# EllarBooher/Syzygy

Hardware: AMD Instinct MI355X
Metric: Mpixels/s deferred-lit+atmosphere (higher is better)
Workload: dtype f32

## Files before the change

syzygy_amd/csrc/kernels_composite.hip:

```cpp

#include "szg_device.hpp"
#include "szg_launch.hpp"

namespace szg
{
namespace
{
template <typename T> SZG_DEV T* row_ptr(const szg_image& im, unsigned y)
{
    return reinterpret_cast<T*>(static_cast<unsigned char*>(im.data) + (size_t)y * im.pitch_bytes);
}

struct SkyLut
{
    const float4* texels;
    int width, height;
    bool finite;
};

SZG_DEV V3 sampleMapDirection(const SkyLut& S, const Atm& a, V3 position, V3 direction)
{
    float const PI = 3.141592653589793f;
    V3 const normalized = normalize(direction);
    float const sinHorizonZenith = a.planetRadius / length(position);
    float const horizonZenith = PI - szg_asinf(sinHorizonZenith);
    float const cosViewZenith = normalized.y;
    float const cosHorizonZenith = -safeSqrt(1.0f - sinHorizonZenith * sinHorizonZenith);
    float const viewZenith = szg_acosf(normalized.y);
    float v;
    if (cosViewZenith > cosHorizonZenith)
    {
        float const angleFraction = viewZenith / horizonZenith;
        v = (1.0f - sqrtf(1.0f - angleFraction)) * 0.5f;
    }
    else
    {
        float const angleFraction = (viewZenith - horizonZenith) / (PI - horizonZenith);
        v = sqrtf(angleFraction) * 0.5f + 0.5f;
    }
    V2 const projectedLight = normalize(V2{-a.incidentDirectionSun.x, -a.incidentDirectionSun.z});
    V2 const projectedView = normalize(V2{direction.x, direction.z});
    float const u = clampf(dot(projectedLight, projectedView), -1.0f, 1.0f) * 0.5f + 0.5f;
    return bilinear_rgb(S.texels, S.width, S.height, (float)S.width, (float)S.height, u, v);
}

SZG_DEV V3 sampleSunDisk(const TLut& L, const Atm& a, V3 position, V3 direction)
{
    V3 const directionToSun = -a.incidentDirectionSun;
    float const cosDirectionSun = dot(direction, directionToSun) / (length(direction) * length(directionToSun));
    float const sinSunRadius = a.sunAngularRadius;
    float const sinDirectionSun = safeSqrt(1.0f - cosDirectionSun * cosDirectionSun);
    if (cosDirectionSun < 0.0f)
    {
        return splat(0.0f);
    }
    V3 const transmittanceToSun = sampleT_Ray(L, a, position, direction);
    return transmittanceToSun * (1.0f - smoothstep(0.2f * sinSunRadius, sinSunRadius, sinDirectionSun));
}

SZG_DEV bool raycastGround(const Atm& a, V3 origin, V3 direction, float& distance)
{
    float t0 = 0.0f, t1 = 0.0f;
    bool const hit = raySphere(origin, direction, a.planetRadius, t0, t1) && t0 > 0.0f;
    distance = t0;
    return hit;
}

SZG_DEV V3 groundSurfaceTerm(const TLut& L, const Atm& a, V3 origin, V3 direction, float distanceToGround)
{
    float const PI = 3.141592653589793f;
    V3 const surfacePosition = origin + distanceToGround * direction;
    V3 const surfaceNormal = normalize(surfacePosition);
    V3 const lightDirection = -a.incidentDirectionSun;
    V3 const viewDirection = -direction;
    V3 const h = normalize(lightDirection + viewDirection);
    float const specularPower = 160.0f;
    float const microfacet = szg_powf(clampf(dot(h, surfaceNormal), 0.0f, 1.0f), specularPower);
    float const normalization = (specularPower + 2.0f) / 8.0f;
    V3 const specular = splat(normalization * microfacet);
    V3 const diffuse = splat(0.4f) / PI;
    V3 const fresnel =
        splat(0.04f) + (splat(1.0f) - splat(0.04f)) * szg_powf(1.0f - clampf(dot(h, lightDirection), 0.0f, 1.0f), 5.0f);
    V3 const albedo = mix(diffuse, specular, fresnel);
    V3 const transmittanceToSun = sampleT_Ray(L, a, surfacePosition, lightDirection);
    V3 const surfaceLuminance = (transmittanceToSun * albedo) * clampf(dot(surfaceNormal, lightDirection), 0.0f, 1.0f);
    V3 const transmittanceToSurface = sampleT_Segment(L, a, origin, surfacePosition);
    return surfaceLuminance * transmittanceToSurface;
}
}

#ifdef SZG_TAIL_DIAG
__device__ unsigned long long* g_tailStamps = nullptr;
extern "C" int szg_debug_tail_buffer(void* d_buffer)
{
    return (int)hipMemcpyToSymbol(HIP_SYMBOL(g_tailStamps), &d_buffer, sizeof d_buffer);
}
struct TailStamp
{
    unsigned long long start;
    unsigned slot;
    SZG_DEV TailStamp(unsigned slot_) : start(wall_clock64()), slot(slot_) {}
// ... 71 lines not shown
    }
    unsigned const gy = global_row(rm, y);

    Atm const a = load_atm(*prep);
#ifdef SZG_EXP_LDS_TLUT
    TLut L = make_tlut(tlut, tW, tH, *prep);
    L.ldsRows = tW == 512 ? (const __attribute__((address_space(3))) float*)s_tlutRows : nullptr;
#else
    TLut const L = make_tlut(tlut, tW, tH, *prep);
#endif
    SkyLut const S{slut, sW, sH, reinterpret_cast<const unsigned*>(slut + (size_t)sW * (size_t)sH)[0] == 0u};
    const szg_camera_packed* cam = cameras + cameraIndex;

    float const sceneDepth = row_ptr<const float>(depth, y)[x];

    V3 position = mk3(cam->position[0], cam->position[1], cam->position[2]) / 1000000.0f;
    position.y *= -1.0f;
    position.y += a.planetRadius;

    float const clipx = ((float)x / (float)drawW - 0.5f) * 2.0f;
    float const clipy = ((float)gy / (float)drawH - 0.5f) * 2.0f;
    M4 const inverseProjection = load_m4(cam->inverseProjection);
    M4 const rotation = load_m4(cam->rotation);
    V4 const dvs = mul(inverseProjection, clipx, clipy, 1.0f, 1.0f);
    V4 const rot = mul(rotation, dvs.x, dvs.y, dvs.z, dvs.w);
    V3 direction = normalize(mk3(rot.x, rot.y, rot.z));
    direction.y *= -1.0f;

    bool isSky = (sceneDepth == 0.0f);
    Material m;
    if (!isSky)
    {
        V4 const diffuse = unpack_half4(row_ptr<const uint2>(g.diffuse, y)[x]);
        V4 const specular = unpack_half4(row_ptr<const uint2>(g.specular, y)[x]);
        V4 const normal = unpack_half4(row_ptr<const uint2>(g.normal, y)[x]);
        V4 const orm = unpack_half4(row_ptr<const uint2>(g.orm, y)[x]);
        float4 const p4 = row_ptr<const float4>(g.position, y)[x];
        m = convertPBR(V4{p4.x, p4.y, p4.z, p4.w}, normal, diffuse, specular, orm);
        isSky = m.position.y > 0.0f;
    }

    V3 surfaceLuminance = splat(0.0f);
    V3 base = splat(0.0f);
    V3 coef = splat(0.0f);
    V3 env2 = splat(0.0f);
    bool hasReflection = false;
    bool march0 = false, march1 = false;
    V3 o0 = position, d0 = direction, o1 = position, d1 = direction;
    float l0 = 0.0f, l1 = 0.0f;

    if (isSky)
    {
        float dtg;
        if (raycastGround(a, position, direction, dtg))
        {
            base = groundSurfaceTerm(L, a, position, direction, dtg);
            march0 = true;
            l0 = dtg;
        }
        else
        {
            base = sampleMapDirection(S, a, position, direction) + sampleSunDisk(L, a, position, direction) * 1.0f;
        }
    }
    else
    {
        uint2 const prior = row_ptr<const uint2>(color, y)[x];
        surfaceLuminance = mk3((float)(prior.x & 0xFFFFu) / 65535.0f, (float)(prior.x >> 16) / 65535.0f,
                               (float)(prior.y & 0xFFFFu) / 65535.0f);

        float shadowFactor = 1.0f;
        if (sunSlot.map != nullptr)
        {
            M4 sm;
#pragma unroll
            for (int k = 0; k < 16; k++)
            {
                sm.m[k] = prep->sunShadow[k];
            }
            V4 c = mul(sm, m.position.x, m.position.y, m.position.z, 1.0f);
            float const w = c.w;
            V3 const coord = mk3(c.x / w, c.y / w, c.z / w);
            V4 const pn = mul(sm, m.normal.x, m.normal.y, m.normal.z, 0.0f);
            float const fdx = sqrtf(1.0f - clampf(pn.x * pn.x, 0.0f, 1.0f));
            float const fdy = sqrtf(1.0f - clampf(pn.y * pn.y, 0.0f, 1.0f));
            shadowFactor = sampleShadowMap(sunSlot.map, sunSlot.width, sunSlot.height, sunSlot.pitchFloats, coord, fdx, fdy);
        }

        m.normal.y *= -1.0f;
        m.position.y *= -1.0f;
        m.position = m.position / 1000000.0f;
        m.position.y += a.planetRadius;

        V3 const surfacePosition = m.position;
        V3 const toSurface = surfacePosition - position;
        bool const samplesLean = waveAll(a.lean && leanRadius2(a, dot(position, position)) && leanRadius2(a, dot(surfacePosition, surfacePosition)) &&
                                         leanLength2(dot(toSurface, toSurface)) &&
                                         leanLength2(dot(a.incidentDirectionSun, a.incidentDirectionSun)));
        V3 const transmittanceToSurface = samplesLean ? sampleT_Segment<true>(L, a, position, surfacePosition)
                                                      : sampleT_Segment<false>(L, a, position, surfacePosition);
        V3 const minusSun = -a.incidentDirectionSun, minusDirection = -direction;
        float const direction2 = dot(minusDirection, minusDirection);
        bool const vectorsLean = samplesLean && waveAll(leanLength2(direction2));
        V3 const lightDirection = vectorsLean ? minusSun * divN0(1.0f, sqrtP(dot(minusSun, minusSun))) : normalize(minusSun);
        V3 const viewDirection = vectorsLean ? minusDirection * divN0(1.0f, sqrtP(direction2)) : normalize(minusDirection);
        float pt0 = 0.0f, pt1 = 0.0f;
        bool const shadowedByPlanet = raySphere(surfacePosition, lightDirection, a.planetRadius, pt0, pt1) && pt0 > 0.0f;
        V3 const halfSum = lightDirection + viewDirection;
        bool const brdfLean = vectorsLean && waveAll(inRange(dot(halfSum, halfSum), 0x1p-40f, 8.0f));
        V3 const brdf = brdfLean ? brdfMix<true>(m, lightDirection, viewDirection) : brdfMix<false>(m, lightDirection, viewDirection);
        V3 const transmittanceToSun = samplesLean ? sampleT_Ray<true>(L, a, surfacePosition, lightDirection)
                                                  : sampleT_Ray<false>(L, a, surfacePosition, lightDirection);
        float const fractionOfSunVisible = vectorsLean ? divN0(a.planetRadius, sqrtP(dot(m.position, m.position)))
                                                       : a.planetRadius / length(m.position);
        float const scalar = (shadowFactor * fractionOfSunVisible) * (shadowedByPlanet ? 0.0f : 1.0f);
        base = ((((scalar * transmittanceToSun) * transmittanceToSurface) * m.occlusion) * brdf) *
               clampf(dot(m.normal, lightDirection), 0.0f, 1.0f);
        l0 = vectorsLean ? sqrtP(dot(toSurface, toSurface)) : length(surfacePosition - position);
        if (FAST)
        {
            base = base + sampleAerial(aerial, (float)x / (float)drawW, (float)gy / (float)drawH, l0);
        }
        else
        {
            march0 = true;
        }

        float const cameraR2 = dot(position, position), surfaceR2 = dot(surfacePosition, surfacePosition);
        float const nBig = 0x1p60f;
        bool const normalFinite = fabsf(m.normal.x) <= nBig && fabsf(m.normal.y) <= nBig && fabsf(m.normal.z) <= nBig;
        float const cameraSinHorizon = vectorsLean ? divN0(a.planetRadius, sqrtP(cameraR2)) : a.planetRadius / length(position);
        bool const aboveGround = cameraSinHorizon <= 1.0f && fractionOfSunVisible <= 1.0f;
        bool const environmentFinite = a.extModerate && a.sunSane && L.moderate && S.finite && normalFinite && aboveGround &&
                                       inRange(cameraR2, a.extFloor2, a.extCeil2) && inRange(surfaceR2, a.extFloor2, a.extCeil2);
        if (m.metallic != 0.0f || !environmentFinite)
        {
            hasReflection = true;
            V3 const negDir = -direction;
            V3 const parallel = dot(m.normal, negDir) * m.normal;
            V3 const reflectionDirection = 2.0f * parallel - negDir;
            coef = (transmittanceToSurface * m.metallic) * computeFresnel(m, negDir, reflectionDirection);
            float dtg2;
            if (raycastGround(a, m.position, reflectionDirection, dtg2))
            {
                env2 = groundSurfaceTerm(L, a, m.position, reflectionDirection, dtg2);
                march1 = true;
                o1 = m.position;
                d1 = reflectionDirection;
                l1 = dtg2;
            }
            else
            {
                env2 = sampleMapDirection(S, a, m.position, reflectionDirection) +
                       sampleSunDisk(L, a, m.position, reflectionDirection) * shadowFactor;
            }
        }
// ... 51 lines not shown
    hasReflection = (flags & 4u) != 0u;
    V3 const ap0 = march0 ? mk3(s_result[0][0][tid], s_result[0][1][tid], s_result[0][2][tid]) : splat(0.0f);
    V3 const ap1 = march1 ? mk3(s_result[1][0][tid], s_result[1][1][tid], s_result[1][2][tid]) : splat(0.0f);
    base = mk3(s_park[0][tid], s_park[1][tid], s_park[2][tid]);
    coef = mk3(s_park[3][tid], s_park[4][tid], s_park[5][tid]);
    env2 = mk3(s_park[6][tid], s_park[7][tid], s_park[8][tid]);
    surfaceLuminance = mk3(s_park[9][tid], s_park[10][tid], s_park[11][tid]);
    V3 transfer = march0 ? (base + ap0) : base;
    if (hasReflection)
    {
        V3 const e2 = march1 ? (env2 + ap1) : env2;
        transfer = transfer + coef * e2;
    }
    V3 const luminance = transfer * mk3(prep->a.sunIntensitySpectrum.x, prep->a.sunIntensitySpectrum.y, prep->a.sunIntensitySpectrum.z);
    V3 const pre = luminance * 10.0f + surfaceLuminance;
    V3 const out = mk3(szg_powf(pre.x, 1.2f), szg_powf(pre.y, 1.2f), szg_powf(pre.z, 1.2f));
    row_ptr<uint2>(color, y)[x] = pack_unorm16x4(out.x, out.y, out.z, 1.0f);
    if (debug.data != nullptr)
    {
        row_ptr<float4>(debug, y)[x] = make_float4(out.x, out.y, out.z, 1.0f);
    }
}

hipError_t launch_composite(hipStream_t s, const szg_scene_texture& scene, unsigned drawW, unsigned drawH, TileArgs tile,
                            const szg_gbuffer& g, ShadowSlot sunSlot, const szg_atmosphere_packed* d_atm, unsigned atmIndex, const szg_camera_packed* d_cam,
                            unsigned camIndex, const szg_directional_light_packed* d_dir, unsigned sunIndex, const float* tlut,
                            unsigned tW, unsigned tH, const float* slut, unsigned sW, unsigned sH, AerialLut aerial, const void* d_prep)
{
    unsigned const rows = tile.nranks <= 1u ? drawH : tile.local_rows;
    if (rows == 0u || drawW == 0u)
    {
// ... 23 lines not shown
```

syzygy_amd/csrc/kernels_deferred.hip:

```cpp

#include "szg_device.hpp"
#include "szg_launch.hpp"

namespace szg
{
namespace
{
SZG_DEV void pixel_of_thread(unsigned& x, unsigned& y)
{
    unsigned const tid = threadIdx.x;
    unsigned const wave = tid >> 6, lane = tid & 63u;
    x = blockIdx.x * 32u + wave * 8u + (lane & 7u);
    y = blockIdx.y * 8u + (lane >> 3);
}
SZG_DEV void pixel_of_thread_bottom_up(unsigned& x, unsigned& y)
{
    unsigned const tid = threadIdx.x;
    unsigned const wave = tid >> 6, lane = tid & 63u;
    x = blockIdx.x * 32u + wave * 8u + (lane & 7u);
    y = (gridDim.y - 1u - blockIdx.y) * 8u + (lane >> 3);
}

template <typename T> SZG_DEV T* row_ptr(const szg_image& im, unsigned y)
{
// ... 454 lines not shown
#endif
    unsigned x, y;
    pixel_of_thread_bottom_up(x, y);
    if (x >= drawW || y >= localRows)
    {
        return;
    }
    V4 const diffuse = unpack_half4(row_ptr<const uint2>(g.diffuse, y)[x]);
    V3 sum = splat(0.0f);
    if (!(diffuse.w < 1.0f))
    {
        V4 const specular = unpack_half4(row_ptr<const uint2>(g.specular, y)[x]);
        V4 const normal = unpack_half4(row_ptr<const uint2>(g.normal, y)[x]);
        V4 const orm = unpack_half4(row_ptr<const uint2>(g.orm, y)[x]);
        float4 const p4 = row_ptr<const float4>(g.position, y)[x];
        Material const m = convertPBR(V4{p4.x, p4.y, p4.z, p4.w}, normal, diffuse, specular, orm);
        const szg_camera_packed* cam = cameras + cameraIndex;
        V3 const viewDirection = normalizeL(mk3(cam->position[0], cam->position[1], cam->position[2]) - m.position);

        float const hi = 0x1p30f;
        bool const positionModerate = fabsf(m.position.x) <= hi && fabsf(m.position.y) <= hi && fabsf(m.position.z) <= hi;
        float const big = 0x1p120f;
        bool const pixelFinite = positionModerate && fabsf(viewDirection.x) <= 2.0f && fabsf(viewDirection.y) <= 2.0f &&
                                 fabsf(viewDirection.z) <= 2.0f && fabsf(m.normal.x) <= big && fabsf(m.normal.y) <= big &&
                                 fabsf(m.normal.z) <= big && fabsf(m.diffuse.x) <= big && fabsf(m.diffuse.y) <= big &&
                                 fabsf(m.diffuse.z) <= big && fabsf(m.reflectance.x) <= big && fabsf(m.reflectance.y) <= big &&
                                 fabsf(m.reflectance.z) <= big && fabsf(m.occlusion) <= big && fabsf(m.normalization) <= big &&
                                 fabsf(m.specularPower) <= big;
        bool const pixelModerate = pixelFinite && fabsf(m.diffuse.x) <= 0x1p16f && fabsf(m.diffuse.y) <= 0x1p16f &&
                                   fabsf(m.diffuse.z) <= 0x1p16f && fabsf(m.reflectance.x) <= 4.0f && fabsf(m.reflectance.y) <= 4.0f &&
                                   fabsf(m.reflectance.z) <= 4.0f && fabsf(m.occlusion) <= 0x1p16f && fabsf(m.normalization) <= 0x1p8f &&
                                   fabsf(m.normal.x) <= 0x1p16f && fabsf(m.normal.y) <= 0x1p16f && fabsf(m.normal.z) <= 0x1p16f;
        bool const waveFinite = waveAll(pixelFinite);
// ... 329 lines not shown
```

syzygy_amd/csrc/kernels_lut.hip:

```cpp

#include "szg_device.hpp"
#include "szg_launch.hpp"

namespace szg
{
template <int CTRL> SZG_DEV float dpp(float v)
{
    return __builtin_bit_cast(float, __builtin_amdgcn_update_dpp(0, __builtin_bit_cast(int, v), CTRL, 0xF, 0xF, false));
}

constexpr int T_LANES = 8;
constexpr int T_STEPS = 500;

template <bool LEAN> SZG_DEV V3 transmittanceProduct(const Atm& a, V3 origin, V3 direction, float distance, float ndt, int sub)
{
    V3 T = splat(1.0f);
    float const rcp500 = rcpN(500.0f);
#pragma unroll 1
    for (int k = 0; k < (T_STEPS + T_LANES - 1) / T_LANES; k++)
    {
        int const i = k * T_LANES + sub;
        float const t = divRX<LEAN>(distance * ((float)i + 0.5f), 500.0f, rcp500);
        V3 const position = origin + t * direction;
        float const altitude = sqrtPX<LEAN>(dotT(position, position)) - a.planetRadius;
// ... 149 lines not shown
        return;
    }
    unsigned const tid = threadIdx.x;
    unsigned const wave = tid >> 6, lane = tid & 63u;
    int const x = (int)(blockIdx.x * 32u + wave * 8u + (lane & 7u));
    int const y = rowBegin + (int)(blockIdx.y * 8u + (lane >> 3));
    if (x >= W || y >= rowEnd)
    {
        return;
    }
    Atm const a = load_atm(*prep);
    TLut const L = make_tlut(tlut, tW, tH, *prep);
    const szg_camera_packed* cam = cameras + cameraIndex;
    float const PI = 3.141592653589793f;

    float const u = ((float)x + 0.5f) / (float)W;
    float const v = ((float)y + 0.5f) / (float)H;

    V3 origin = mk3(cam->position[0], cam->position[1], cam->position[2]) / 1000000.0f;
    origin.y *= -1.0f;
    origin.y += a.planetRadius;

    float const radius = length(origin);
    float const sinHorizonZenith = a.planetRadius / radius;
    float const horizonZenith = PI - szg_asinf(sinHorizonZenith);
    float const cosineViewLightProjected = (u - 0.5f) * 2.0f;
    V2 const lightDirectionProjected = normalize(V2{-a.incidentDirectionSun.x, -a.incidentDirectionSun.z});
    float azimuthSun = szg_asinf(lightDirectionProjected.x);
    if (lightDirectionProjected.y < 0.0f)
    {
        azimuthSun = PI - azimuthSun;
    }
    float const azimuth = szg_acosf(clampf(cosineViewLightProjected, -1.0f, 1.0f)) + azimuthSun;
    float viewZenith;
    float const unnormalized_v = 2.0f * v - 1.0f;
    if (v < 0.5f)
    {
        float const angleFraction = 1.0f - unnormalized_v * unnormalized_v;
        viewZenith = angleFraction * horizonZenith;
    }
    else
    {
        float const angleFraction = unnormalized_v * unnormalized_v;
        viewZenith = (PI - horizonZenith) * angleFraction + horizonZenith;
    }
    float const elevation = -(viewZenith - PI / 2.0f);

    float const ce = szg_cosf(elevation);
    V3 const direction = normalize(mk3(szg_sinf(azimuth) * ce, szg_sinf(elevation), szg_cosf(azimuth) * ce));

    float const distance = raycastAtmosphere(a, origin, direction);
    V3 const luminance = scatteringIntegral(L, a, origin, direction, distance);
    lut[y * W + x] = make_float4(luminance.x, luminance.y, luminance.z, 1.0f);
    if (!slutTexelFinite(luminance.x, luminance.y, luminance.z))
    {
        atomicOr(reinterpret_cast<unsigned*>(lut + (size_t)W * (size_t)H), 1u);
    }
}

__global__ __launch_bounds__(256) void k_slut_check(float4* __restrict__ lut, unsigned n)
{
    unsigned const id = blockIdx.x * 256u + threadIdx.x;
    bool ok = true;
    if (id < n)
    {
        float4 const t = lut[id];
// ... 309 lines not shown
```

syzygy_amd/csrc/szg_device.hpp:

```cpp
#pragma once

#include <hip/hip_fp16.h>
#include <hip/hip_runtime.h>

#include "szg/abi.h"
#include "szg/fpmath.h"

#define SZG_DEV __device__ __forceinline__

namespace szg
{
struct V2
{
    float x, y;
};
struct V3
{
    float x, y, z;
};
struct V4
{
    float x, y, z, w;
};

// ... 116 lines not shown
    u = __builtin_fmaf(u, s, 0.166666671633720397949219f);
    u = __builtin_fmaf(u, s, 0.5f);
    u = __builtin_fmaf(s * s, u, s) + 1.0f;
    return __builtin_ldexpf(u, (int)q);
}
template <bool LEAN> SZG_DEV float divX(float a, float b) { return LEAN ? divR0(a, b, rcpN(b)) : a / b; }
template <bool LEAN> SZG_DEV float divRX(float a, float b, float y) { return LEAN ? divR0(a, b, y) : a / b; }
SZG_DEV float xorSign(float x, unsigned signMask)
{
    return __builtin_bit_cast(float, __builtin_bit_cast(unsigned, x) ^ signMask);
}
SZG_DEV bool slutTexelFinite(float r, float g, float b) { return fabsf(r) <= 0x1p100f && fabsf(g) <= 0x1p100f && fabsf(b) <= 0x1p100f; }
SZG_DEV bool inRange(float x, float lo, float hi) { return x >= lo && x <= hi; }
SZG_DEV float divN0(float a, float b) { return divR0(a, b, rcpN(b)); }
SZG_DEV bool waveAll(bool c) { return __builtin_amdgcn_ballot_w64(!c) == 0ull; }

SZG_DEV float powLean(float x, float y)
{
    int const bits = szg_float_to_bits(x * 1.3333333333333333333333333333333333333f);
    int const e = ((bits >> 23) & 0xFF) - 127;
    float const m = szg_bits_to_float(szg_float_to_bits(x) - (e << 23));
    float const t = szg_div_moderate(m - 1.0f, m + 1.0f);
    float const t2 = t * t;
    float p = 0.2392828464508056640625f;
    p = __builtin_fmaf(p, t2, 0.28518211841583251953125f);
    p = __builtin_fmaf(p, t2, 0.400005877017974853515625f);
    p = __builtin_fmaf(p, t2, 0.666666686534881591796875f);
    p = __builtin_fmaf(p, t2, 2.0f);
    float const fe = (float)e;
    float const lg = __builtin_fmaf(t, p, 0.693147180559945286226764f * fe);
// ... 298 lines not shown
    if (LEAN && a.zeroAbsorptionRayleigh && a.zeroScatteringOzone)
    {
        e.extinction = (scatteringRayleigh + scatteringMie) + absorptionOzone;
    }
    else if (LEAN && a.zeroAbsorptionRayleigh)
    {
        e.extinction = ((scatteringRayleigh + scatteringMie) + scatteringOzone) + absorptionOzone;
    }
    else
    {
        e.extinction = scatteringRayleigh + absorptionRayleigh + scatteringMie + absorptionMie + scatteringOzone + absorptionOzone;
    }
    return e;
}

SZG_DEV bool raySphere(V3 f, V3 d, float radius, float& t0, float& t1)
{
    float const b = -1.0f * dotA(f, d);
    V3 const chord = f + b * d;
    float const discriminant = radius * radius - dotA(chord, chord);
    float const c = dotA(f, f) - radius * radius;
    if (discriminant < 0.0f)
    {
        return false;
    }
    float q = b;
    float const s = sqrtf(discriminant);
    q = (b < 0.0f) ? (q - s) : (q + s);
    float a0 = c / q;
    float a1 = q;
    if (a0 > a1)
    {
        float const tmp = a0;
        a0 = a1;
        a1 = tmp;
    }
    t0 = a0;
    t1 = a1;
    return true;
}

SZG_DEV float raycastAtmosphere(const Atm& a, V3 origin, V3 direction)
{
    float at0 = 0.0f, at1 = 0.0f;
    bool const hitAtmosphere = raySphere(origin, direction, a.atmosphereRadius, at0, at1) && at1 > 0.0f;
    at0 = fmaxf(0.0f, at0);
    float pt0 = 0.0f, pt1 = 0.0f;
    bool const hitPlanet = raySphere(origin, direction, a.planetRadius, pt0, pt1) && pt0 > 0.0f;
    if (hitPlanet)
    {
        at1 = fminf(pt0, at1);
    }
    return hitAtmosphere ? (at1 - at0) : 0.0f;
}

struct TLut
{
    const float4* texels;
    int width, height;
    float fwidth, fheight;
    float u_bias, u_scale, v_bias, v_scale;
    bool moderate;
    bool rowsInterior;
// ... 274 lines not shown
        return segmentRatio<true>(L, a, pf, dotA(from, direction), lenFrom, pt, dotA(to, direction), lenTo, sqrtP(dotA(direction, direction)));
    }
    V3 const direction = normalizeA(to - from);
    float const lenFrom = lengthA(from);
    float const lenTo = lengthA(to);
    RadiusPart const pf = radiusPart<false>(L, a, lenFrom);
    RadiusPart const pt = radiusPart<false>(L, a, lenTo);
    return segmentRatio<false>(L, a, pf, dotA(from, direction), lenFrom, pt, dotA(to, direction), lenTo, lengthA(direction));
}

SZG_DEV float phaseRayleigh(float cosine)
{
    float const scalar = 3.0f / (16.0f * 3.141592653589793f);
    return scalar * (1.0f + cosine * cosine);
}
SZG_DEV float phaseMie(float cosine, float g)
{
    float const scalar = 3.0f / (8.0f * 3.141592653589793f);
    float const numerator = (1.0f - g * g) * (1.0f + cosine * cosine);
    float const denominator = (2.0f + g * g) * szg_powf(1.0f + g * g - 2.0f * g * cosine, 1.5f);
    return scalar * numerator / denominator;
}

struct MarchSetup
{
    V3 origin, scatteringDir;
    float dS, pR, pM, sin_sunRadius, cos_sunRadius;
    float mu_sunAndStep, r_mu, two_r_mu, r2, r_musun;
    bool up;
    bool extLean;
    bool sunClear;
    bool firstStepOnly;
    bool belowOzone;
    V3 T_origin;
};

// ... 108 lines not shown
        m.scatteringDir = -(direction * divN0(1.0f, lenDirection));
        radius = sqrtP(origin2);
        mu = divN0(dotA(origin, direction), radius * lenDirection);
        mu_sun = divN0(dotA(origin, toSun), radius * a.sunLengthLean);
    }
    else
    {
        m.scatteringDir = -normalizeA(direction);
        radius = lengthA(origin);
        mu = dotA(origin, direction) / (lengthA(origin) * lengthA(direction));
        mu_sun = dotA(origin, toSun) / (lengthA(origin) * a.sunLength);
    }

    float const incidentCosine = dotA(a.incidentDirectionSun, m.scatteringDir);
    m.pR = phaseRayleigh(incidentCosine);
    m.pM = phaseMie(incidentCosine, 0.8f);
    m.sin_sunRadius = a.sinSunRadius;
    m.cos_sunRadius = a.cosSunRadius;

    m.mu_sunAndStep = safeSqrt(mu_sun * mu - safeSqrt((1.0f - mu_sun * mu_sun) * (1.0f - mu * mu)));
    m.r_mu = radius * mu;
    m.two_r_mu = 2.0f * radius * mu;
    m.r2 = radius * radius;
    m.r_musun = radius * mu_sun;
    m.up = mu > 0.0f;
    m.T_origin = setupLean ? sampleT_RadiusMu<true>(L, a, radius, m.up ? mu : -mu) : sampleT_RadiusMu<false>(L, a, radius, m.up ? mu : -mu);
    m.dS = sampleDistance / 32.0f;

    float const L2 = SZG_CON(SZG_C_STEP, m.two_r_mu, sampleDistance, sampleDistance * sampleDistance) + m.r2;
    float const tStar = -m.r_mu;
    float const rmin2 = (tStar > 0.0f && tStar < sampleDistance) ? m.r2 * (1.0f - mu * mu) : fminf(m.r2, L2);
    bool const lean = a.lean && rmin2 >= a.leanFloor2 && inRange(radius, 0x1p-30f, 0x1p30f) && inRange(sampleDistance, 0.0f, 0x1p30f) &&
                      m.sin_sunRadius >= 0x1p-30f && leanLength2(sun2) && leanLength2(direction2) && fabsf(mu) <= 2.0f &&
                      fabsf(mu_sun) <= 2.0f;
    m.extLean = waveAll(a.extModerate && rmin2 >= a.extFloor2 && fmaxf(m.r2, L2) <= a.extCeil2);
    m.firstStepOnly = waveAll(lean && m.dS >= 0.0000001f);
    {
        float const ozoneLow = a.planetRadius + 0.0099f;
        m.belowOzone = waveAll(lean && fmaxf(m.r2, L2) <= ozoneLow * ozoneLow);
    }
    {
        float const rMax = sqrtf(fmaxf(m.r2, L2));
        m.sunClear = waveAll(lean && m.cos_sunRadius >= 0.0f && m.sin_sunRadius > 0.0f && m.r_musun > 0.0f &&
                             m.r_musun * 0.999f >= (1.25f * m.sin_sunRadius + 0x1p-10f) * rMax);
    }
    if (waveAll(lean))
    {
        if (waveAll(fmaxf(m.r2, L2) <= a.innerCeil2))
        {
            return marchLoop<true, true>(L, a, m);
        }
        return marchLoop<true, false>(L, a, m);
    }
    return marchLoop<false>(L, a, m);
}

struct Material
{
    V3 position;
    V3 normal;
    V3 subscattering;
    V3 reflectance;
    float occlusion;
    float specularPower;
    float metallic;
    V3 diffuse;
    float normalization;
};

SZG_DEV Material convertPBR(V4 position, V4 normal, V4 diffuse, V4 specular, V4 orm)
{
    Material m;
    V3 const spec = mk3(specular.x, specular.y, specular.z);
    float const mx = fmaxf(fmaxf(spec.x, spec.y), spec.z);
    V3 const metallicReflectance = (splat(0.5f) * spec) / mx;
    m.position = mk3(position.x, position.y, position.z);
    m.normal = mk3(normal.x, normal.y, normal.z);
    m.subscattering = mk3(diffuse.x, diffuse.y, diffuse.z);
    m.metallic = orm.z;
    m.reflectance = mix(splat(0.04f), metallicReflectance, splat(m.metallic));
    m.occlusion = orm.x;
    m.specularPower = szg_powf(160.0f, 1.0f - orm.y);
    m.diffuse = m.subscattering / 3.14159265359f;
    m.normalization = (m.specularPower + 2.0f) / 8.0f;
    return m;
}

template <bool LEAN = false> SZG_DEV V3 brdfMix(const Material& m, V3 lightDir, V3 viewDir)
{
    V3 const hs = lightDir + viewDir;
    float const hd = dotP(hs, hs);
    V3 const h = hs * divX<LEAN>(1.0f, sqrtX<LEAN>(hd));
    float const microfacet = szg_powf(clampf(dotP(h, m.normal), 0.0f, 1.0f), m.specularPower);
    V3 const specular = splat(m.normalization * microfacet);
    float const p = szg_powf(1.0f - clampf(dotP(h, lightDir), 0.0f, 1.0f), 5.0f);
    V3 const fresnel = m.reflectance + (splat(1.0f) - m.reflectance) * p;
    return mix(m.diffuse, specular, fresnel);
}

SZG_DEV V3 computeFresnel(const Material& m, V3 lightOutgoing, V3 viewOutgoing)
{
    V3 const h = normalizeP(lightOutgoing + viewOutgoing);
    float const p = szg_powf(1.0f - clampf(dotP(h, lightOutgoing), 0.0f, 1.0f), 5.0f);
    return m.reflectance + (splat(1.0f) - m.reflectance) * p;
}

SZG_DEV float sampleShadowMap(const float* __restrict__ map, unsigned W, unsigned H, unsigned pitchFloats, V3 coord, float fdx,
                              float fdy)
{
    float const fragmentDepth = coord.z;
    float const fW = (float)(int)W;
    float const fH = (float)(int)H;
    float const dx = 1.5f * fdx / fW;
    float const dy = 1.5f * fdy / fH;
    float summed = 0.0f;
#pragma unroll
    for (int y = -2; y <= 2; y++)
    {
// ... 23 lines not shown
```

Baseline: 2475.

## Add wave-uniform fast-math paths for division, sqrt, normalize and pow across composite kernels

Adds lean variants of division, sqrt, normalize, pow and smoothstep across the sky, sun disk, ground, PBR, BRDF, Fresnel, phase function and tonemap code. Each variant is taken only when a wave-wide ballot confirms the operands sit in safe ranges, so the slower IEEE-correct sequences are avoided in the common case. Constant divisions are replaced by multiplication with precomputed reciprocals. The cost is extra range checks and ballots, larger code and possible register pressure, plus small accuracy differences.

```diff
diff --git a/syzygy_amd/csrc/kernels_composite.hip b/syzygy_amd/csrc/kernels_composite.hip
--- a/syzygy_amd/csrc/kernels_composite.hip
+++ b/syzygy_amd/csrc/kernels_composite.hip
@@ -18,28 +18,42 @@
     bool finite;
 };
 
+
 SZG_DEV V3 sampleMapDirection(const SkyLut& S, const Atm& a, V3 position, V3 direction)
 {
     float const PI = 3.141592653589793f;
-    V3 const normalized = normalize(direction);
-    float const sinHorizonZenith = a.planetRadius / length(position);
+    V2 const sunHorizontal = V2{-a.incidentDirectionSun.x, -a.incidentDirectionSun.z};
+    V2 const viewHorizontal = V2{direction.x, direction.z};
+    float const direction2 = dot(direction, direction), position2 = dot(position, position);
+    float const sunHorizontal2 = dot(sunHorizontal, sunHorizontal), viewHorizontal2 = dot(viewHorizontal, viewHorizontal);
+    bool const lean = waveAll(inRange(a.planetRadius, 0x1p-30f, 0x1p30f) && leanLength2(direction2) && leanLength2(position2) &&
+                              leanLength2(sunHorizontal2) && leanLength2(viewHorizontal2));
+    V3 const normalized = lean ? direction * rsqrtLean(direction2) : normalize(direction);
+    float const sinHorizonZenith = lean ? divN0(a.planetRadius, sqrtP(position2)) : a.planetRadius / length(position);
     float const horizonZenith = PI - szg_asinf(sinHorizonZenith);
     float const cosViewZenith = normalized.y;
-    float const cosHorizonZenith = -safeSqrt(1.0f - sinHorizonZenith * sinHorizonZenith);
+    float const cosRadicand = fmaxf(1.0f - sinHorizonZenith * sinHorizonZenith, 0.0f);
+    float const cosHorizonZenith = -(lean ? sqrtN(cosRadicand) : sqrtf(cosRadicand));
     float const viewZenith = szg_acosf(normalized.y);
-    float v;
-    if (cosViewZenith > cosHorizonZenith)
-    {
-        float const angleFraction = viewZenith / horizonZenith;
-        v = (1.0f - sqrtf(1.0f - angleFraction)) * 0.5f;
+    bool const above = cosViewZenith > cosHorizonZenith;
+    float const numerator = above ? viewZenith : (viewZenith - horizonZenith);
+    float const denominator = above ? horizonZenith : (PI - horizonZenith);
+    float const angleFraction = waveAll(divNumOK(numerator) && divDenOK(denominator)) ? divN(numerator, denominator) : numerator / denominator;
+    float const radicand = above ? (1.0f - angleFraction) : angleFraction;
+    float const root = waveAll(sqrtArgOK(radicand)) ? sqrtN(radicand) : sqrtf(radicand);
+    float const v = above ? ((1.0f - root) * 0.5f) : (root * 0.5f + 0.5f);
+    V2 projectedLight, projectedView;
+    if (lean)
+    {
+        float const sl = rsqrtLean(sunHorizontal2), sv = rsqrtLean(viewHorizontal2);
+        projectedLight = V2{sunHorizontal.x * sl, sunHorizontal.y * sl};
+        projectedView = V2{viewHorizontal.x * sv, viewHorizontal.y * sv};
     }
     else
     {
-        float const angleFraction = (viewZenith - horizonZenith) / (PI - horizonZenith);
-        v = sqrtf(angleFraction) * 0.5f + 0.5f;
-    }
-    V2 const projectedLight = normalize(V2{-a.incidentDirectionSun.x, -a.incidentDirectionSun.z});
-    V2 const projectedView = normalize(V2{direction.x, direction.z});
+        projectedLight = normalize(sunHorizontal);
+        projectedView = normalize(viewHorizontal);
+    }
     float const u = clampf(dot(projectedLight, projectedView), -1.0f, 1.0f) * 0.5f + 0.5f;
     return bilinear_rgb(S.texels, S.width, S.height, (float)S.width, (float)S.height, u, v);
 }
@@ -47,21 +61,31 @@
 SZG_DEV V3 sampleSunDisk(const TLut& L, const Atm& a, V3 position, V3 direction)
 {
     V3 const directionToSun = -a.incidentDirectionSun;
-    float const cosDirectionSun = dot(direction, directionToSun) / (length(direction) * length(directionToSun));
+    float const direction2 = dot(direction, direction), sun2 = dot(directionToSun, directionToSun);
+    float const cosNumerator = dot(direction, directionToSun);
+    bool const lean = waveAll(leanLength2(direction2) && leanLength2(sun2) && divNumOK(cosNumerator));
+    float const cosDirectionSun =
+        lean ? divN0(cosNumerator, sqrtP(direction2) * sqrtP(sun2)) : cosNumerator / (length(direction) * length(directionToSun));
     float const sinSunRadius = a.sunAngularRadius;
-    float const sinDirectionSun = safeSqrt(1.0f - cosDirectionSun * cosDirectionSun);
+    float const sinRadicand = fmaxf(1.0f - cosDirectionSun * cosDirectionSun, 0.0f);
+    float const sinDirectionSun = lean ? sqrtN(sinRadicand) : sqrtf(sinRadicand);
     if (cosDirectionSun < 0.0f)
     {
         return splat(0.0f);
     }
-    V3 const transmittanceToSun = sampleT_Ray(L, a, position, direction);
-    return transmittanceToSun * (1.0f - smoothstep(0.2f * sinSunRadius, sinSunRadius, sinDirectionSun));
+    bool const sampleLean = waveAll(a.lean && leanRadius2(a, dotA(position, position)) && leanLength2(dotA(direction, direction)) &&
+                                    divNumOK(dotA(position, direction)));
+    V3 const transmittanceToSun = sampleLean ? sampleT_Ray<true>(L, a, position, direction) : sampleT_Ray<false>(L, a, position, direction);
+    float const edge0 = 0.2f * sinSunRadius;
+    bool const stepLean = waveAll(divNumOK(sinDirectionSun - edge0) && divDenOK(sinSunRadius - edge0));
+    float const disk = stepLean ? smoothstepLean(edge0, sinSunRadius, sinDirectionSun) : smoothstep(edge0, sinSunRadius, sinDirectionSun);
+    return transmittanceToSun * (1.0f - disk);
 }
 
 SZG_DEV bool raycastGround(const Atm& a, V3 origin, V3 direction, float& distance)
 {
     float t0 = 0.0f, t1 = 0.0f;
-    bool const hit = raySphere(origin, direction, a.planetRadius, t0, t1) && t0 > 0.0f;
+    bool const hit = raySphere<true>(origin, direction, a.planetRadius, t0, t1) && t0 > 0.0f;
     distance = t0;
     return hit;
 }
@@ -70,21 +94,31 @@
 {
     float const PI = 3.141592653589793f;
     V3 const surfacePosition = origin + distanceToGround * direction;
-    V3 const surfaceNormal = normalize(surfacePosition);
     V3 const lightDirection = -a.incidentDirectionSun;
     V3 const viewDirection = -direction;
-    V3 const h = normalize(lightDirection + viewDirection);
+    V3 const halfSum = lightDirection + viewDirection;
+    float const surface2 = dot(surfacePosition, surfacePosition), half2 = dot(halfSum, halfSum);
+    bool const vectorsLean = waveAll(leanLength2(surface2) && leanLength2(half2));
+    V3 const surfaceNormal = vectorsLean ? surfacePosition * rsqrtLean(surface2) : normalize(surfacePosition);
+    V3 const h = vectorsLean ? halfSum * rsqrtLean(half2) : normalize(halfSum);
     float const specularPower = 160.0f;
-    float const microfacet = szg_powf(clampf(dot(h, surfaceNormal), 0.0f, 1.0f), specularPower);
+    float const baseSpecular = clampf(dot(h, surfaceNormal), 0.0f, 1.0f);
+    float const baseFresnel = 1.0f - clampf(dot(h, lightDirection), 0.0f, 1.0f);
+    bool const powsLean = waveAll(powLeanOK(baseSpecular, specularPower) && powLeanOK(baseFresnel, 5.0f));
+    float const microfacet = powsLean ? powLean(baseSpecular, specularPower) : szg_powf(baseSpecular, specularPower);
     float const normalization = (specularPower + 2.0f) / 8.0f;
     V3 const specular = splat(normalization * microfacet);
     V3 const diffuse = splat(0.4f) / PI;
-    V3 const fresnel =
-        splat(0.04f) + (splat(1.0f) - splat(0.04f)) * szg_powf(1.0f - clampf(dot(h, lightDirection), 0.0f, 1.0f), 5.0f);
+    V3 const fresnel = splat(0.04f) + (splat(1.0f) - splat(0.04f)) * (powsLean ? powLean(baseFresnel, 5.0f) : szg_powf(baseFresnel, 5.0f));
     V3 const albedo = mix(diffuse, specular, fresnel);
-    V3 const transmittanceToSun = sampleT_Ray(L, a, surfacePosition, lightDirection);
+    V3 const toSurface = surfacePosition - origin;
+    bool const samplesLean = waveAll(a.lean && leanRadius2(a, dotA(origin, origin)) && leanRadius2(a, dotA(surfacePosition, surfacePosition)) &&
+                                     leanLength2(dotA(toSurface, toSurface)) && leanLength2(a.sun2));
+    V3 const transmittanceToSun = samplesLean ? sampleT_Ray<true>(L, a, surfacePosition, lightDirection)
+                                              : sampleT_Ray<false>(L, a, surfacePosition, lightDirection);
     V3 const surfaceLuminance = (transmittanceToSun * albedo) * clampf(dot(surfaceNormal, lightDirection), 0.0f, 1.0f);
-    V3 const transmittanceToSurface = sampleT_Segment(L, a, origin, surfacePosition);
+    V3 const transmittanceToSurface = samplesLean ? sampleT_Segment<true>(L, a, origin, surfacePosition)
+                                                  : sampleT_Segment<false>(L, a, origin, surfacePosition);
     return surfaceLuminance * transmittanceToSurface;
 }
 }
@@ -186,17 +220,24 @@
 
     float const sceneDepth = row_ptr<const float>(depth, y)[x];
 
-    V3 position = mk3(cam->position[0], cam->position[1], cam->position[2]) / 1000000.0f;
+    V3 const cameraPosition = mk3(cam->position[0], cam->position[1], cam->position[2]);
+    V3 position = waveAll(divNumOK(cameraPosition)) ? divR(cameraPosition, 1000000.0f, kRcp1e6) : cameraPosition / 1000000.0f;
     position.y *= -1.0f;
     position.y += a.planetRadius;
 
-    float const clipx = ((float)x / (float)drawW - 0.5f) * 2.0f;
-    float const clipy = ((float)gy / (float)drawH - 0.5f) * 2.0f;
+    float const fdrawW = (float)drawW, fdrawH = (float)drawH;
+    bool const extentsLean = extentLean(drawW) && extentLean(drawH);
+    float const screenx = extentsLean ? divR0((float)x, fdrawW, rcpN(fdrawW)) : (float)x / fdrawW;
+    float const screeny = extentsLean ? divR0((float)gy, fdrawH, rcpN(fdrawH)) : (float)gy / fdrawH;
+    float const clipx = (screenx - 0.5f) * 2.0f;
+    float const clipy = (screeny - 0.5f) * 2.0f;
     M4 const inverseProjection = load_m4(cam->inverseProjection);
     M4 const rotation = load_m4(cam->rotation);
     V4 const dvs = mul(inverseProjection, clipx, clipy, 1.0f, 1.0f);
     V4 const rot = mul(rotation, dvs.x, dvs.y, dvs.z, dvs.w);
-    V3 direction = normalize(mk3(rot.x, rot.y, rot.z));
+    V3 const rotated = mk3(rot.x, rot.y, rot.z);
+    float const rotated2 = dot(rotated, rotated);
+    V3 direction = waveAll(leanLength2(rotated2)) ? rotated * rsqrtLean(rotated2) : normalize(rotated);
     direction.y *= -1.0f;
 
     bool isSky = (sceneDepth == 0.0f);
@@ -208,7 +249,7 @@
         V4 const normal = unpack_half4(row_ptr<const uint2>(g.normal, y)[x]);
         V4 const orm = unpack_half4(row_ptr<const uint2>(g.orm, y)[x]);
         float4 const p4 = row_ptr<const float4>(g.position, y)[x];
-        m = convertPBR(V4{p4.x, p4.y, p4.z, p4.w}, normal, diffuse, specular, orm);
+        m = convertPBR<true>(V4{p4.x, p4.y, p4.z, p4.w}, normal, diffuse, specular, orm);
         isSky = m.position.y > 0.0f;
     }
 
@@ -238,8 +279,8 @@
     else
     {
         uint2 const prior = row_ptr<const uint2>(color, y)[x];
-        surfaceLuminance = mk3((float)(prior.x & 0xFFFFu) / 65535.0f, (float)(prior.x >> 16) / 65535.0f,
-                               (float)(prior.y & 0xFFFFu) / 65535.0f);
+        surfaceLuminance = mk3(divR0((float)(prior.x & 0xFFFFu), 65535.0f, kRcp65535), divR0((float)(prior.x >> 16), 65535.0f, kRcp65535),
+                               divR0((float)(prior.y & 0xFFFFu), 65535.0f, kRcp65535));
 
         float shadowFactor = 1.0f;
         if (sunSlot.map != nullptr)
@@ -252,16 +293,25 @@
             }
             V4 c = mul(sm, m.position.x, m.position.y, m.position.z, 1.0f);
             float const w = c.w;
-            V3 const coord = mk3(c.x / w, c.y / w, c.z / w);
+            V3 coord;
+            if (waveAll(divDenOK(w) && divNumOK(mk3(c.x, c.y, c.z))))
+            {
+                float const yw = rcpN(w);
+                coord = mk3(divR(c.x, w, yw), divR(c.y, w, yw), divR(c.z, w, yw));
+            }
+            else
+            {
+                coord = mk3(c.x / w, c.y / w, c.z / w);
+            }
             V4 const pn = mul(sm, m.normal.x, m.normal.y, m.normal.z, 0.0f);
-            float const fdx = sqrtf(1.0f - clampf(pn.x * pn.x, 0.0f, 1.0f));
-            float const fdy = sqrtf(1.0f - clampf(pn.y * pn.y, 0.0f, 1.0f));
+            float const fdx = sqrtN(1.0f - clampf(pn.x * pn.x, 0.0f, 1.0f));
+            float const fdy = sqrtN(1.0f - clampf(pn.y * pn.y, 0.0f, 1.0f));
             shadowFactor = sampleShadowMap(sunSlot.map, sunSlot.width, sunSlot.height, sunSlot.pitchFloats, coord, fdx, fdy);
         }
 
         m.normal.y *= -1.0f;
         m.position.y *= -1.0f;
-        m.position = m.position / 1000000.0f;
+        m.position = waveAll(divNumOK(m.position)) ? divR(m.position, 1000000.0f, kRcp1e6) : m.position / 1000000.0f;
         m.position.y += a.planetRadius;
 
         V3 const surfacePosition = m.position;
@@ -277,7 +327,7 @@
         V3 const lightDirection = vectorsLean ? minusSun * divN0(1.0f, sqrtP(dot(minusSun, minusSun))) : normalize(minusSun);
         V3 const viewDirection = vectorsLean ? minusDirection * divN0(1.0f, sqrtP(direction2)) : normalize(minusDirection);
         float pt0 = 0.0f, pt1 = 0.0f;
-        bool const shadowedByPlanet = raySphere(surfacePosition, lightDirection, a.planetRadius, pt0, pt1) && pt0 > 0.0f;
+        bool const shadowedByPlanet = raySphere<true>(surfacePosition, lightDirection, a.planetRadius, pt0, pt1) && pt0 > 0.0f;
         V3 const halfSum = lightDirection + viewDirection;
         bool const brdfLean = vectorsLean && waveAll(inRange(dot(halfSum, halfSum), 0x1p-40f, 8.0f));
         V3 const brdf = brdfLean ? brdfMix<true>(m, lightDirection, viewDirection) : brdfMix<false>(m, lightDirection, viewDirection);
@@ -291,7 +341,7 @@
         l0 = vectorsLean ? sqrtP(dot(toSurface, toSurface)) : length(surfacePosition - position);
         if (FAST)
         {
-            base = base + sampleAerial(aerial, (float)x / (float)drawW, (float)gy / (float)drawH, l0);
+            base = base + sampleAerial(aerial, screenx, screeny, l0);
         }
         else
         {
@@ -311,7 +361,7 @@
             V3 const negDir = -direction;
             V3 const parallel = dot(m.normal, negDir) * m.normal;
             V3 const reflectionDirection = 2.0f * parallel - negDir;
-            coef = (transmittanceToSurface * m.metallic) * computeFresnel(m, negDir, reflectionDirection);
+            coef = (transmittanceToSurface * m.metallic) * computeFresnel<true>(m, negDir, reflectionDirection);
             float dtg2;
             if (raycastGround(a, m.position, reflectionDirection, dtg2))
             {
@@ -393,7 +443,9 @@
     }
     V3 const luminance = transfer * mk3(prep->a.sunIntensitySpectrum.x, prep->a.sunIntensitySpectrum.y, prep->a.sunIntensitySpectrum.z);
     V3 const pre = luminance * 10.0f + surfaceLuminance;
-    V3 const out = mk3(szg_powf(pre.x, 1.2f), szg_powf(pre.y, 1.2f), szg_powf(pre.z, 1.2f));
+    bool const tonemapLean = waveAll(powLeanOK(pre.x, 1.2f) && powLeanOK(pre.y, 1.2f) && powLeanOK(pre.z, 1.2f));
+    V3 const out = tonemapLean ? mk3(powLean(pre.x, 1.2f), powLean(pre.y, 1.2f), powLean(pre.z, 1.2f))
+                               : mk3(szg_powf(pre.x, 1.2f), szg_powf(pre.y, 1.2f), szg_powf(pre.z, 1.2f));
     row_ptr<uint2>(color, y)[x] = pack_unorm16x4(out.x, out.y, out.z, 1.0f);
     if (debug.data != nullptr)
     {
diff --git a/syzygy_amd/csrc/kernels_deferred.hip b/syzygy_amd/csrc/kernels_deferred.hip
--- a/syzygy_amd/csrc/kernels_deferred.hip
+++ b/syzygy_amd/csrc/kernels_deferred.hip
@@ -492,9 +492,11 @@
         V4 const normal = unpack_half4(row_ptr<const uint2>(g.normal, y)[x]);
         V4 const orm = unpack_half4(row_ptr<const uint2>(g.orm, y)[x]);
         float4 const p4 = row_ptr<const float4>(g.position, y)[x];
-        Material const m = convertPBR(V4{p4.x, p4.y, p4.z, p4.w}, normal, diffuse, specular, orm);
+        Material const m = convertPBR<true>(V4{p4.x, p4.y, p4.z, p4.w}, normal, diffuse, specular, orm);
         const szg_camera_packed* cam = cameras + cameraIndex;
-        V3 const viewDirection = normalizeL(mk3(cam->position[0], cam->position[1], cam->position[2]) - m.position);
+        V3 const toCamera = mk3(cam->position[0], cam->position[1], cam->position[2]) - m.position;
+        float const toCamera2 = dotL(toCamera, toCamera);
+        V3 const viewDirection = waveAll(leanLength2(toCamera2)) ? toCamera * rsqrtLean(toCamera2) : normalizeL(toCamera);
 
         float const hi = 0x1p30f;
         bool const positionModerate = fabsf(m.position.x) <= hi && fabsf(m.position.y) <= hi && fabsf(m.position.z) <= hi;
diff --git a/syzygy_amd/csrc/kernels_lut.hip b/syzygy_amd/csrc/kernels_lut.hip
--- a/syzygy_amd/csrc/kernels_lut.hip
+++ b/syzygy_amd/csrc/kernels_lut.hip
@@ -187,18 +187,25 @@
     const szg_camera_packed* cam = cameras + cameraIndex;
     float const PI = 3.141592653589793f;
 
-    float const u = ((float)x + 0.5f) / (float)W;
-    float const v = ((float)y + 0.5f) / (float)H;
-
-    V3 origin = mk3(cam->position[0], cam->position[1], cam->position[2]) / 1000000.0f;
+    float const fW = (float)W, fH = (float)H;
+    bool const extentsLean = extentLean((unsigned)W) && extentLean((unsigned)H);
+    float const u = extentsLean ? divR0((float)x + 0.5f, fW, rcpN(fW)) : ((float)x + 0.5f) / fW;
+    float const v = extentsLean ? divR0((float)y + 0.5f, fH, rcpN(fH)) : ((float)y + 0.5f) / fH;
+
+    V3 const cameraPosition = mk3(cam->position[0], cam->position[1], cam->position[2]);
+    V3 origin = waveAll(divNumOK(cameraPosition)) ? divR(cameraPosition, 1000000.0f, kRcp1e6) : cameraPosition / 1000000.0f;
     origin.y *= -1.0f;
     origin.y += a.planetRadius;
 
-    float const radius = length(origin);
-    float const sinHorizonZenith = a.planetRadius / radius;
+    V2 const sunHorizontal = V2{-a.incidentDirectionSun.x, -a.incidentDirectionSun.z};
+    float const origin2 = dot(origin, origin), sunHorizontal2 = dot(sunHorizontal, sunHorizontal);
+    bool const frameLean = waveAll(inRange(a.planetRadius, 0x1p-30f, 0x1p30f) && leanLength2(origin2) && leanLength2(sunHorizontal2));
+    float const radius = frameLean ? sqrtP(origin2) : length(origin);
+    float const sinHorizonZenith = frameLean ? divN0(a.planetRadius, radius) : a.planetRadius / radius;
     float const horizonZenith = PI - szg_asinf(sinHorizonZenith);
     float const cosineViewLightProjected = (u - 0.5f) * 2.0f;
-    V2 const lightDirectionProjected = normalize(V2{-a.incidentDirectionSun.x, -a.incidentDirectionSun.z});
+    float const sunScale = frameLean ? rsqrtLean(sunHorizontal2) : 1.0f / sqrtf(sunHorizontal2);
+    V2 const lightDirectionProjected = V2{sunHorizontal.x * sunScale, sunHorizontal.y * sunScale};
     float azimuthSun = szg_asinf(lightDirectionProjected.x);
     if (lightDirectionProjected.y < 0.0f)
     {
@@ -220,9 +227,11 @@
     float const elevation = -(viewZenith - PI / 2.0f);
 
     float const ce = szg_cosf(elevation);
-    V3 const direction = normalize(mk3(szg_sinf(azimuth) * ce, szg_sinf(elevation), szg_cosf(azimuth) * ce));
-
-    float const distance = raycastAtmosphere(a, origin, direction);
+    V3 const unnormalized = mk3(szg_sinf(azimuth) * ce, szg_sinf(elevation), szg_cosf(azimuth) * ce);
+    float const unnormalized2 = dot(unnormalized, unnormalized);
+    V3 const direction = waveAll(leanLength2(unnormalized2)) ? unnormalized * rsqrtLean(unnormalized2) : normalize(unnormalized);
+
+    float const distance = raycastAtmosphere<true>(a, origin, direction);
     V3 const luminance = scatteringIntegral(L, a, origin, direction, distance);
     lut[y * W + x] = make_float4(luminance.x, luminance.y, luminance.z, 1.0f);
     if (!slutTexelFinite(luminance.x, luminance.y, luminance.z))
diff --git a/syzygy_amd/csrc/szg_device.hpp b/syzygy_amd/csrc/szg_device.hpp
--- a/syzygy_amd/csrc/szg_device.hpp
+++ b/syzygy_amd/csrc/szg_device.hpp
@@ -154,6 +154,22 @@
 SZG_DEV bool inRange(float x, float lo, float hi) { return x >= lo && x <= hi; }
 SZG_DEV float divN0(float a, float b) { return divR0(a, b, rcpN(b)); }
 SZG_DEV bool waveAll(bool c) { return __builtin_amdgcn_ballot_w64(!c) == 0ull; }
+
+constexpr float kRcp1e6 = 0x1.0c6f7ap-20f;
+constexpr float kRcp65535 = 0x1.0001p-16f;
+constexpr float kRcpPi = 0x1.45f306p-2f;
+SZG_DEV bool divNumOK(float a) { return inRange(fabsf(a), 0x1p-60f, 0x1p60f) || a == 0.0f; }
+SZG_DEV bool divNumOK(V3 v) { return divNumOK(v.x) && divNumOK(v.y) && divNumOK(v.z); }
+SZG_DEV bool divDenOK(float b) { return inRange(fabsf(b), 0x1p-60f, 0x1p60f); }
+SZG_DEV bool sqrtArgOK(float x) { return inRange(x, 0x1p-96f, 3.4028235e38f) || x == 0.0f; }
+SZG_DEV V3 divR(V3 v, float b, float y) { return V3{divR(v.x, b, y), divR(v.y, b, y), divR(v.z, b, y)}; }
+SZG_DEV float rsqrtLean(float d2) { return rcpN(sqrtP(d2)); }
+SZG_DEV bool extentLean(unsigned n) { return n >= 1u && n <= 16384u; }
+SZG_DEV float smoothstepLean(float e0, float e1, float x)
+{
+    float const t = clampf(divN0(x - e0, e1 - e0), 0.0f, 1.0f);
+    return t * t * (3.0f - 2.0f * t);
+}
 
 SZG_DEV float powLean(float x, float y)
 {
@@ -482,7 +498,7 @@
     return e;
 }
 
-SZG_DEV bool raySphere(V3 f, V3 d, float radius, float& t0, float& t1)
+template <bool TRY = false> SZG_DEV bool raySphere(V3 f, V3 d, float radius, float& t0, float& t1)
 {
     float const b = -1.0f * dotA(f, d);
     V3 const chord = f + b * d;
@@ -493,9 +509,9 @@
         return false;
     }
     float q = b;
-    float const s = sqrtf(discriminant);
+    float const s = (TRY && waveAll(sqrtArgOK(discriminant))) ? sqrtN(discriminant) : sqrtf(discriminant);
     q = (b < 0.0f) ? (q - s) : (q + s);
-    float a0 = c / q;
+    float a0 = (TRY && waveAll(divNumOK(c) && divDenOK(q))) ? divN(c, q) : c / q;
     float a1 = q;
     if (a0 > a1)
     {
@@ -508,13 +524,13 @@
     return true;
 }
 
-SZG_DEV float raycastAtmosphere(const Atm& a, V3 origin, V3 direction)
+template <bool TRY = false> SZG_DEV float raycastAtmosphere(const Atm& a, V3 origin, V3 direction)
 {
     float at0 = 0.0f, at1 = 0.0f;
-    bool const hitAtmosphere = raySphere(origin, direction, a.atmosphereRadius, at0, at1) && at1 > 0.0f;
+    bool const hitAtmosphere = raySphere<TRY>(origin, direction, a.atmosphereRadius, at0, at1) && at1 > 0.0f;
     at0 = fmaxf(0.0f, at0);
     float pt0 = 0.0f, pt1 = 0.0f;
-    bool const hitPlanet = raySphere(origin, direction, a.planetRadius, pt0, pt1) && pt0 > 0.0f;
+    bool const hitPlanet = raySphere<TRY>(origin, direction, a.planetRadius, pt0, pt1) && pt0 > 0.0f;
     if (hitPlanet)
     {
         at1 = fminf(pt0, at1);
@@ -819,12 +835,13 @@
     float const scalar = 3.0f / (16.0f * 3.141592653589793f);
     return scalar * (1.0f + cosine * cosine);
 }
-SZG_DEV float phaseMie(float cosine, float g)
+template <bool LEAN = false> SZG_DEV float phaseMie(float cosine, float g)
 {
     float const scalar = 3.0f / (8.0f * 3.141592653589793f);
     float const numerator = (1.0f - g * g) * (1.0f + cosine * cosine);
-    float const denominator = (2.0f + g * g) * szg_powf(1.0f + g * g - 2.0f * g * cosine, 1.5f);
-    return scalar * numerator / denominator;
+    float const base = 1.0f + g * g - 2.0f * g * cosine;
+    float const denominator = (2.0f + g * g) * (LEAN ? powLean(base, 1.5f) : szg_powf(base, 1.5f));
+    return LEAN ? divN0(scalar * numerator, denominator) : scalar * numerator / denominator;
 }
 
 struct MarchSetup
@@ -963,11 +980,16 @@
 
     float const incidentCosine = dotA(a.incidentDirectionSun, m.scatteringDir);
     m.pR = phaseRayleigh(incidentCosine);
-    m.pM = phaseMie(incidentCosine, 0.8f);
+    m.pM = waveAll(fabsf(incidentCosine) <= 1.02f) ? phaseMie<true>(incidentCosine, 0.8f) : phaseMie<false>(incidentCosine, 0.8f);
     m.sin_sunRadius = a.sinSunRadius;
     m.cos_sunRadius = a.cosSunRadius;
 
-    m.mu_sunAndStep = safeSqrt(mu_sun * mu - safeSqrt((1.0f - mu_sun * mu_sun) * (1.0f - mu * mu)));
+    {
+        float const inner = fmaxf((1.0f - mu_sun * mu_sun) * (1.0f - mu * mu), 0.0f);
+        bool const innerLean = waveAll(fabsf(mu) <= 2.0f && fabsf(mu_sun) <= 2.0f && sqrtArgOK(inner));
+        float const outer = fmaxf(mu_sun * mu - (innerLean ? sqrtN(inner) : sqrtf(inner)), 0.0f);
+        m.mu_sunAndStep = (innerLean && waveAll(sqrtArgOK(outer))) ? sqrtN(outer) : sqrtf(outer);
+    }
     m.r_mu = radius * mu;
     m.two_r_mu = 2.0f * radius * mu;
     m.r2 = radius * radius;
@@ -989,7 +1011,7 @@
         m.belowOzone = waveAll(lean && fmaxf(m.r2, L2) <= ozoneLow * ozoneLow);
     }
     {
-        float const rMax = sqrtf(fmaxf(m.r2, L2));
+        float const rMax = setupLean ? sqrtP(fmaxf(m.r2, L2)) : sqrtf(fmaxf(m.r2, L2));
         m.sunClear = waveAll(lean && m.cos_sunRadius >= 0.0f && m.sin_sunRadius > 0.0f && m.r_musun > 0.0f &&
                              m.r_musun * 0.999f >= (1.25f * m.sin_sunRadius + 0x1p-10f) * rMax);
     }
@@ -1017,20 +1039,31 @@
     float normalization;
 };
 
-SZG_DEV Material convertPBR(V4 position, V4 normal, V4 diffuse, V4 specular, V4 orm)
+template <bool TRY = false> SZG_DEV Material convertPBR(V4 position, V4 normal, V4 diffuse, V4 specular, V4 orm)
 {
     Material m;
     V3 const spec = mk3(specular.x, specular.y, specular.z);
     float const mx = fmaxf(fmaxf(spec.x, spec.y), spec.z);
-    V3 const metallicReflectance = (splat(0.5f) * spec) / mx;
+    V3 const halfSpec = splat(0.5f) * spec;
+    V3 metallicReflectance;
+    if (TRY && waveAll(divDenOK(mx) && divNumOK(halfSpec)))
+    {
+        float const y = rcpN(mx);
+        metallicReflectance = V3{divR(halfSpec.x, mx, y), divR(halfSpec.y, mx, y), divR(halfSpec.z, mx, y)};
+    }
+    else
+    {
+        metallicReflectance = halfSpec / mx;
+    }
     m.position = mk3(position.x, position.y, position.z);
     m.normal = mk3(normal.x, normal.y, normal.z);
     m.subscattering = mk3(diffuse.x, diffuse.y, diffuse.z);
     m.metallic = orm.z;
     m.reflectance = mix(splat(0.04f), metallicReflectance, splat(m.metallic));
     m.occlusion = orm.x;
-    m.specularPower = szg_powf(160.0f, 1.0f - orm.y);
-    m.diffuse = m.subscattering / 3.14159265359f;
+    float const glossiness = 1.0f - orm.y;
+    m.specularPower = (TRY && waveAll(powLeanOK(160.0f, glossiness))) ? powLean(160.0f, glossiness) : szg_powf(160.0f, glossiness);
+    m.diffuse = (TRY && waveAll(divNumOK(m.subscattering))) ? divR(m.subscattering, 3.14159265359f, kRcpPi) : m.subscattering / 3.14159265359f;
     m.normalization = (m.specularPower + 2.0f) / 8.0f;
     return m;
 }
@@ -1040,17 +1073,23 @@
     V3 const hs = lightDir + viewDir;
     float const hd = dotP(hs, hs);
     V3 const h = hs * divX<LEAN>(1.0f, sqrtX<LEAN>(hd));
-    float const microfacet = szg_powf(clampf(dotP(h, m.normal), 0.0f, 1.0f), m.specularPower);
+    float const baseSpecular = clampf(dotP(h, m.normal), 0.0f, 1.0f);
+    float const baseFresnel = 1.0f - clampf(dotP(h, lightDir), 0.0f, 1.0f);
+    bool const powsLean = LEAN && waveAll(powLeanOK(baseSpecular, m.specularPower) && powLeanOK(baseFresnel, 5.0f));
+    float const microfacet = powsLean ? powLean(baseSpecular, m.specularPower) : szg_powf(baseSpecular, m.specularPower);
     V3 const specular = splat(m.normalization * microfacet);
-    float const p = szg_powf(1.0f - clampf(dotP(h, lightDir), 0.0f, 1.0f), 5.0f);
+    float const p = powsLean ? powLean(baseFresnel, 5.0f) : szg_powf(baseFresnel, 5.0f);
     V3 const fresnel = m.reflectance + (splat(1.0f) - m.reflectance) * p;
     return mix(m.diffuse, specular, fresnel);
 }
 
-SZG_DEV V3 computeFresnel(const Material& m, V3 lightOutgoing, V3 viewOutgoing)
-{
-    V3 const h = normalizeP(lightOutgoing + viewOutgoing);
-    float const p = szg_powf(1.0f - clampf(dotP(h, lightOutgoing), 0.0f, 1.0f), 5.0f);
+template <bool TRY = false> SZG_DEV V3 computeFresnel(const Material& m, V3 lightOutgoing, V3 viewOutgoing)
+{
+    V3 const hs = lightOutgoing + viewOutgoing;
+    float const hd = dotP(hs, hs);
+    V3 const h = (TRY && waveAll(leanLength2(hd))) ? hs * rsqrtLean(hd) : normalizeP(hs);
+    float const base = 1.0f - clampf(dotP(h, lightOutgoing), 0.0f, 1.0f);
+    float const p = (TRY && waveAll(powLeanOK(base, 5.0f))) ? powLean(base, 5.0f) : szg_powf(base, 5.0f);
     return m.reflectance + (splat(1.0f) - m.reflectance) * p;
 }
 
```

New measurement: 2486 (median of 6 runs). No clear change (+0.5%).
